# ktiwary2/nerf_pl

Hardware: AMD Instinct MI355X
Metric: rays/sec (64c+128f) Blender-lego 400^2 training step (higher is better)
Workload: dtype f16x3

## Files before the change

__graft_entry__.py:

```python
import os
import subprocess
import sys

REPO = os.path.dirname(os.path.abspath(__file__))


def build() -> None:
    jobs = str(min(16, os.cpu_count() or 1))
    subprocess.run(["make", "-C", REPO, "-j", jobs], check=True)
    r = subprocess.run(["make", "-C", REPO, "-j", jobs, "asan"], check=False)
    if r.returncode != 0:
        print(f"build(): optional `make asan` failed (rc {r.returncode}); "
              "tests/test_abi_asan.py will skip", file=sys.stderr)
    if REPO not in sys.path:
        sys.path.insert(0, REPO)
    import nerf_pl_amd
    from nerf_pl_amd import (_lib, _lib_mesh, _lib_mesh_normals, _lib_optim, _lib_posegrad,
                             _lib_raygrad)
    missing = (_lib.missing_symbols() + _lib_mesh.missing_symbols()
               + _lib_mesh_normals.missing_symbols() + _lib_raygrad.missing_symbols()
               + _lib_posegrad.missing_symbols() + _lib_optim.missing_symbols())
    if missing:
        raise RuntimeError(f"libnerf_pl_amd.so lacks {missing}")


def smoke() -> None:
    if REPO not in sys.path:
        sys.path.insert(0, REPO)
    import torch
    from nerf_pl_amd import Embedding, NeRF, ReplayRNG, render_rays
    from nerf_pl_amd.rays import blender_rays
    from oracle import nerf_oracle as O

    dev = torch.device("cuda", 0)
    n_rays, S, I = 64, 32, 32
    rays = blender_rays(16, 1, near=2.0, far=6.0)[:n_rays].contiguous()
    g = torch.Generator().manual_seed(0)
    draws = [torch.rand(n_rays, S, generator=g), torch.randn(n_rays, S, generator=g),
             torch.rand(n_rays, I, generator=g), torch.rand(n_rays, I, generator=g),
             torch.randn(n_rays, S + I, generator=g)]
    params = [O.make_params(1, sigma_bias=0.5), O.make_params(2, sigma_bias=0.5)]
    ocap, cap = {}, {}
    ref = O.render_rays(params, rays, S, False, 1.0, 1.0, I, 32768, False,
                        rng=O.ReplayRNG(draws), capture=ocap)
# ... 26 lines not shown
```

nerf_pl_amd/csrc/mlp_fwd3.hip:

```cpp
#include "x3.h"

namespace {

using namespace x3;

constexpr int kHeadBytes = NR_H_SIZE * 4;
constexpr int kHeadDma = (kHeadBytes + 1023) / 1024;
constexpr int kHeadLds = kHeadDma * 1024;
#define NR_PE_REGS (NR_F16 || NR_BF1)
constexpr int kPeQ = 12;
constexpr int kPeBytes = NR_PE_REGS ? 0 : kWaves * kPeQ * 64 * 16;
constexpr int kNS = 2;
constexpr int kBlocks = kWaves;
constexpr int kLdsBytes = kRingBytes + kHeadLds + kPeBytes;
static_assert(kLdsBytes <= 160 * 1024, "LDS budget");

constexpr int kL1 = 0, kL2 = 4, kL3 = 20, kL4 = 36, kL5 = 52, kL6 = 72, kL7 = 88, kL8 = 104;
constexpr int kFinal = 120, kDir = 136, kQAll = 145, kQSigma = 120;

struct FwdTab {
    __host__ __device__ static constexpr int64_t off(int q) {
        return (int64_t)kHeadBytes + (int64_t)q * kSlotBytes;
    }
    __host__ __device__ static constexpr int sg(int q) { return q < kDir ? q / 2 : kDir / 2 + (q - kDir); }
    __host__ __device__ static constexpr int first(int G) { return G < kDir / 2 ? 2 * G : kDir + (G - kDir / 2); }
    __host__ __device__ static constexpr int size(int G) { return G < kDir / 2 ? 2 : 1; }
};
static_assert(FwdTab::off(kQAll) == (NR_F16 ? 2388000 : (NR_BF1 ? 1200160 : 3575840)),
              "packed size must match packing.fwd3_offsets()");

template <bool RELU, int NF, int NS>
__device__ __forceinline__ void head_dot(const f32x4 (&acc)[NF][NS], const float* __restrict__ w,
                                         int g, float (&p)[2]) {
    p[0] = p[1] = 0.f;
#pragma unroll
    for (int F = 0; F < NF; ++F) {
        const f32x4 v = *reinterpret_cast<const f32x4*>(w + 16 * F + 4 * g);
#pragma unroll
        for (int S = 0; S < NS; ++S)
#pragma unroll
            for (int r = 0; r < 4; ++r) p[S] = fmaf(RELU ? relu_keep(acc[F][S][r]) : acc[F][S][r], v[r], p[S]);
    }
#pragma unroll
    for (int S = 0; S < NS; ++S) p[S] = sum_over_groups(p[S]);
}

__device__ __forceinline__ void pe_encode(float (&pe)[16], float px, float py, float pz, int g) {
#pragma unroll
    for (int s = 0; s < 2; ++s)
#pragma unroll
        for (int i = 0; i < 4; ++i) {
            const int m = 4 * (4 * s + g) + i;
            const int k = (m * 11) >> 5;
            const int c = m - 3 * k;
            const float v = c == 0 ? px : (c == 1 ? py : pz);
            float sn, cs;
            sincosf(v * __uint_as_float((uint32_t)(127 + k) << 23), &sn, &cs);
            pe[8 * s + i] = sn;
            pe[8 * s + 4 + i] = cs;
        }
    if (g == 3) {
        pe[10] = px; pe[11] = py; pe[14] = pz; pe[15] = 0.f;
    }
}

__device__ __forceinline__ void pe_gather(float (&pe)[16], const float* __restrict__ row, int g) {
#pragma unroll
    for (int s = 0; s < 2; ++s)
#pragma unroll
        for (int i = 0; i < 4; ++i) {
            const int m = min(4 * (4 * s + g) + i, 29);
            const int k = (m * 11) >> 5;
            const int c = m - 3 * k;
            pe[8 * s + i] = row[3 + 6 * k + c];
            pe[8 * s + 4 + i] = row[6 + 6 * k + c];
        }
    if (g == 3) {
        pe[10] = row[0]; pe[11] = row[1]; pe[14] = row[2]; pe[15] = 0.f;
    }
}

__device__ __forceinline__ void dir_encode(float (&d)[8], float dx, float dy, float dz, int g) {
    const float sc = __uint_as_float((uint32_t)(127 + g) << 23);
    sincosf(dx * sc, &d[0], &d[4]);
    sincosf(dy * sc, &d[1], &d[5]);
    sincosf(dz * sc, &d[2], &d[6]);
    d[3] = g == 0 ? dx : (g == 1 ? dy : (g == 2 ? dz : 0.f));
    d[7] = 0.f;
}

__device__ __forceinline__ void dir_gather(float (&d)[8], const float* __restrict__ row, int g) {
#pragma unroll
    for (int c = 0; c < 3; ++c) {
        d[c] = row[3 + 6 * g + c];
        d[4 + c] = row[6 + 6 * g + c];
    }
    d[3] = g < 3 ? row[min(g, 2)] : 0.f;
    d[7] = 0.f;
}

template <int W, bool ROWS>
__device__ __forceinline__ void store_pe4(const float* v, int s, int jh, int S, int g,
                                          float* __restrict__ blk, int lane) {
    const int T = 2 * s + (g >> 1), gp = 2 * (g & 1) + jh;
#if NR_BF1
    store_slot(f32x4{v[0], v[1], v[2], v[3]}, blk, (T * 2 + S) * 64 + 16 * gp + (lane & 15));
#else
    if constexpr (ROWS)
        *reinterpret_cast<f32x4*>(blk + (16 * S + (lane & 15)) * W + 16 * T + 4 * gp) =
            f32x4{v[0], v[1], v[2], v[3]};
    else
// ... 24 lines not shown
template <bool SAVE>
struct DirPeSide {
    static constexpr int before(int T) { return SAVE ? T / 2 : 0; }
    const float (&dpe)[kNS][8];
    float* dst;
    int g, lane;
    template <typename GC>
    __device__ __forceinline__ void operator()(GC, int t) const {
        if constexpr (SAVE) {
            if (t & 1) {
                const int u = t >> 1;
                store_pe4<32, true>(&dpe[u >> 1][4 * (u & 1)], 0, u & 1, u >> 1, g, dst, lane);
            }
        }
    }
};

struct Fwd3Args {
    const char* packed;
    const float* pts; const float* rays; const float* z; const float* x;
    int n, spr, xstride;
    float* out; float* save;
    const int32_t* slist; const int32_t* scount;
};

template <bool RELU, bool STORE, bool MASK, bool SIG, bool ROWS = true>
struct AccU {
    static constexpr bool kStores = STORE;
    static constexpr bool kPaired = STORE && ROWS && kRowPair;
    template <typename P> __device__ __forceinline__ void begin(const P&) {}
    const f32x4 (&X)[16][kNS];
    float* dst;
    uint32_t* msk;
    const float* wsig;
    int lane, g;
    float pend[2] = {0.f, 0.f};
    f32x4 held = {0.f, 0.f, 0.f, 0.f};
    uint32_t w[4] = {0u, 0u, 0u, 0u};
    float sig[2] = {0.f, 0.f};
    f32x2 wsg[2][4];
    __device__ __forceinline__ f32x2 wsig_of(int s, int p) const {
        return *reinterpret_cast<const f32x2*>(wsig + 32 * s + 16 * (p >> 1) + 4 * g + 2 * (p & 1));
    }
    __device__ __forceinline__ void preload() {
        if constexpr (SIG)
#pragma unroll
// ... 45 lines not shown
    const float (&pe)[kNS][N];
    template <typename SC>
    __device__ __forceinline__ void operator()(SC, int sb, int p, float& x0, float& x1) const {
        constexpr int s = SC::value;
        x0 = pe[sb][8 * s + 2 * p];
        x1 = pe[sb][8 * s + 2 * p + 1];
    }
};

template <int S = 0, typename GetU>
__device__ __forceinline__ void drain_all(GetU& u) {
    if constexpr (S < 8) {
#pragma unroll
        for (int sb = 0; sb < kNS; ++sb)
#pragma unroll
            for (int p = 0; p < 4; ++p) {
                float x0, x1;
                u(IC<S>(), sb, p, x0, x1);
            }
        drain_all<S + 1>(u);
    }
}

template <int MODE, bool SIGMA_ONLY, bool SAVE, bool LIST = false>
__global__ void __launch_bounds__(64 * kWaves, 1) mlp_fwd3_kernel(Fwd3Args a) {
    constexpr bool EMB = MODE == FWD_EMB;
    constexpr int QEND = SIGMA_ONLY ? kQSigma : kQAll;
    static_assert(!LIST || (SAVE && MODE == FWD_RAYS), "a listed run saves, on the ray path");
    __shared__ __attribute__((aligned(16))) char smem[kLdsBytes];
    const int lane = threadIdx.x & 63;
    const int wave = __builtin_amdgcn_readfirstlane(threadIdx.x >> 6);
    const int g = lane >> 4;
    const int blk = blockIdx.x * kBlocks + wave;
    const int m = LIST ? __builtin_amdgcn_readfirstlane(*a.scount) : a.n;
    if (LIST && (int)blockIdx.x * kBlocks * 32 >= m) return;
    int smp[2];
    bool valid[2];
#pragma unroll
    for (int S = 0; S < kNS; ++S) {
        const int s_raw = blk * 32 + 16 * S + (lane & 15);
        valid[S] = s_raw < m;
        if constexpr (LIST) smp[S] = a.slist[valid[S] ? s_raw : 0];
        else smp[S] = valid[S] ? s_raw : a.n - 1;
    }
    const char* P = a.packed;

    float pe[kNS][16], dg[kNS][8];
    float in[kNS][7];
#pragma unroll
    for (int S = 0; S < kNS; ++S) {
        const int s = smp[S];
        if constexpr (EMB) {
            pe_gather(pe[S], a.x + (size_t)s * a.xstride, g);
            if constexpr (!SIGMA_ONLY) dir_gather(dg[S], a.x + (size_t)s * a.xstride + NR_XYZ_CH, g);
        } else if constexpr (MODE == FWD_PTS) {
#pragma unroll
            for (int c = 0; c < 3; ++c) in[S][c] = a.pts[(size_t)s * 3 + c];
        } else {
            const float* r = a.rays + (size_t)(s / a.spr) * 8;
#pragma unroll
            for (int c = 0; c < 6; ++c) in[S][c] = r[c];
            in[S][6] = a.z[s];
        }
    }

    float* Hs = reinterpret_cast<float*>(smem + kRingBytes);
    const Dma dma = make_dma(P, FwdTab::off(kQAll), smem, wave, lane);
#pragma unroll
    for (int i = wave; i < kHeadDma; i += kWaves)
        __builtin_amdgcn_raw_ptr_buffer_load_lds(
            dma.rsrc, (__attribute__((address_space(3))) void*)(smem + kRingBytes + i * 1024), 16,
            dma.voff, i * 1024, 0, 0);
    prologue<FwdTab, QEND>(dma);
    const float* H = Hs;
    const int nb = (int)nr_blocks_pad(a.n);
    float* const SV = a.save;

    [[maybe_unused]] f32x4* pe_lds =
        reinterpret_cast<f32x4*>(smem + kRingBytes + kHeadLds) + wave * kPeQ * 64 + lane;
#pragma unroll
    for (int S = 0; S < kNS; ++S) {
        if constexpr (MODE == FWD_PTS) {
            pe_encode(pe[S], in[S][0], in[S][1], in[S][2], g);
        } else if constexpr (MODE == FWD_RAYS) {
            const float zz = in[S][6];
            pe_encode(pe[S], nr_add(in[S][0], nr_mul(in[S][3], zz)),
                      nr_add(in[S][1], nr_mul(in[S][4], zz)), nr_add(in[S][2], nr_mul(in[S][5], zz)), g);
            if constexpr (!SIGMA_ONLY) dir_encode(dg[S], in[S][3], in[S][4], in[S][5], g);
        }
    }
#if !NR_PE_REGS
#pragma unroll
    for (int q = 0; q < 8; ++q)
        pe_lds[q * 64] = f32x4{pe[q >> 2][4 * (q & 3)], pe[q >> 2][4 * (q & 3) + 1],
                               pe[q >> 2][4 * (q & 3) + 2], pe[q >> 2][4 * (q & 3) + 3]};
    if constexpr (!SIGMA_ONLY) {
#pragma unroll
        for (int S = 0; S < 2; ++S) {
            pe_lds[(8 + 2 * S) * 64] = f32x4{dg[S][0], dg[S][1], dg[S][2], dg[S][3]};
            pe_lds[(9 + 2 * S) * 64] = f32x4{dg[S][4], dg[S][5], dg[S][6], dg[S][7]};
        }
    }
#endif

    Ahead f0;
    enter<FwdTab, 0, QEND>(smem, lane, f0);

    ActN<kNS> A, B;
    Pieces b[kNS];
    auto hseg = [&](int l) { return SV + nr_sv_h(l, nb) + (size_t)blk * NR_SEGF(256); };
    NoSide none;
// ... 168 lines not shown
#elif NR_BF1
#define NR_FWD3_BYTES_NAME nr_fwd3_packed_bytes_b1
#else
#define NR_FWD3_BYTES_NAME nr_fwd3_packed_bytes
#endif
NR_API int64_t NR_FWD3_BYTES_NAME(void) { return FwdTab::off(kQAll); }

NR_API int NR_X3_NAME(nr_pack)(const float* flat, const int32_t* map, int64_t n, const int32_t* head_map,
                      void* out, void* stream) {
    NR_REQUIRE(n == (FwdTab::off(kQAll) - kHeadBytes) / 2, "nr_pack_x3: map has %lld entries, "
               "expected %lld", (long long)n, (long long)((FwdTab::off(kQAll) - kHeadBytes) / 2));
    NR_REQUIRE(flat && map && head_map && out, "nr_pack_x3: null pointer");
    pack3_kernel<<<(unsigned)((n + 255) / 256), 256, 0, (hipStream_t)stream>>>(
        flat, map, n, head_map, reinterpret_cast<char*>(out));
    NR_LAUNCH_CHECK("nr_pack_x3");
    return 0;
}

NR_API int NR_X3_NAME(nr_mlp_fwd)(const void* packed, const float* rays, const float* z, int64_t n,
                         int samples_per_ray, const float* x, int xstride, int sigma_only,
                         float* out, float* save, void* stream) {
    NR_REQUIRE(n >= 0 && n < (int64_t)1 << 31, "nr_mlp_fwd_x3: n=%lld out of range", (long long)n);
    if (n == 0) return 0;
    NR_REQUIRE(packed && out, "nr_mlp_fwd_x3: null packed/out");
    NR_REQUIRE(((uintptr_t)packed & 15) == 0 && ((uintptr_t)out & 15) == 0 &&
                   ((uintptr_t)save & 15) == 0,
               "nr_mlp_fwd_x3: packed/out/save must be 16-byte aligned");
    const bool emb = x != nullptr;
    if (emb) {
        NR_REQUIRE(xstride >= (sigma_only ? NR_XYZ_CH : NR_XYZ_CH + NR_DIR_CH),
                   "nr_mlp_fwd_x3: xstride %d too small", xstride);
    } else {
        NR_REQUIRE(rays && z && samples_per_ray > 0, "nr_mlp_fwd_x3: rays/z/samples_per_ray");
    }
    NR_REQUIRE(!(sigma_only && save && emb),
               "nr_mlp_fwd_x3: a sigma_only run keeps activations only on the ray path");
    Fwd3Args a{reinterpret_cast<const char*>(packed), nullptr, rays, z, x, (int)n,
               samples_per_ray, xstride, out, save};
    const int blocks = (int)((n + 32 * kBlocks - 1) / (32 * kBlocks));
    hipStream_t st = (hipStream_t)stream;
    const bool sv = save != nullptr;
    if (emb) {
        if (sigma_only) mlp_fwd3_kernel<FWD_EMB, true, false><<<blocks, 64 * kWaves, 0, st>>>(a);
        else if (sv) mlp_fwd3_kernel<FWD_EMB, false, true><<<blocks, 64 * kWaves, 0, st>>>(a);
        else mlp_fwd3_kernel<FWD_EMB, false, false><<<blocks, 64 * kWaves, 0, st>>>(a);
    } else {
        if (sigma_only && sv) mlp_fwd3_kernel<FWD_RAYS, true, true><<<blocks, 64 * kWaves, 0, st>>>(a);
        else if (sigma_only) mlp_fwd3_kernel<FWD_RAYS, true, false><<<blocks, 64 * kWaves, 0, st>>>(a);
        else if (sv) mlp_fwd3_kernel<FWD_RAYS, false, true><<<blocks, 64 * kWaves, 0, st>>>(a);
        else mlp_fwd3_kernel<FWD_RAYS, false, false><<<blocks, 64 * kWaves, 0, st>>>(a);
    }
    NR_LAUNCH_CHECK("nr_mlp_fwd_x3");
    return 0;
}

#if !NR_BF1
NR_API int NR_X3_NAME(nr_mlp_fwd_listed)(const void* packed, const float* rays, const float* z,
                                         int64_t n, int samples_per_ray, int sigma_only,
                                         float* save, const int32_t* samples,
                                         const int32_t* count, void* stream) {
    NR_REQUIRE(n >= 0 && n < (int64_t)1 << 31, "nr_mlp_fwd_listed: n=%lld out of range", (long long)n);
    if (n == 0) return 0;
    NR_REQUIRE(packed && rays && z && save && samples && count && samples_per_ray > 0,
               "nr_mlp_fwd_listed: null pointer or samples_per_ray");
    NR_REQUIRE(((uintptr_t)packed & 15) == 0 && ((uintptr_t)save & 15) == 0,
               "nr_mlp_fwd_listed: packed/save must be 16-byte aligned");
    Fwd3Args a{reinterpret_cast<const char*>(packed), nullptr, rays, z, nullptr, (int)n,
               samples_per_ray, 0, nullptr, save, samples, count};
    const int blocks = (int)((n + 32 * kBlocks - 1) / (32 * kBlocks));
    hipStream_t st = (hipStream_t)stream;
    if (sigma_only) mlp_fwd3_kernel<FWD_RAYS, true, true, true><<<blocks, 64 * kWaves, 0, st>>>(a);
    else mlp_fwd3_kernel<FWD_RAYS, false, true, true><<<blocks, 64 * kWaves, 0, st>>>(a);
    NR_LAUNCH_CHECK("nr_mlp_fwd_listed");
    return 0;
}
#endif

NR_API int NR_X3_NAME(nr_mlp_sigma_points)(const void* packed, const float* pts, int64_t n,
                                  float* sigma_out, void* stream) {
// ... 12 lines not shown
```

nerf_pl_amd/csrc/probe.hip:

```cpp
#include "layout.h"

NR_API int64_t nr_layout_query(int what) {
    switch (what) {
        case 0: return NR_F_TOTAL;
        case 1: return NR_F_HEAD;
        case 2: return NR_B_TOTAL;
        case 3: return NR_SAVE_PER_BLOCK;
        case 4: return NR_GRAD_PER_BLOCK;
        case 5: return NR_H_SIZE;
        case 6: return NR_F_L5;
        case 7: return NR_F_DIR;
        case 8: return NR_B_L5T;
        case 9: return 2;
        default: return -1;
    }
}

namespace {
__global__ void probe_mfma_kernel(const float* a_in, const float* b_in, float* d_out) {
    const int l = threadIdx.x;
    const float a = a_in[(l & 31) * 2 + (l >> 5)];
    const float b = b_in[(l >> 5) * 32 + (l & 31)];
    f32x16 c = {};
    c = nr_mfma32(a, b, c);
    for (int r = 0; r < 16; ++r) d_out[nr_acc_row(r, l >> 5) * 32 + (l & 31)] = c[r];
}

__global__ void probe_rand_kernel(uint64_t seed, uint32_t stream, uint64_t idx0, int64_t n,
                                  float* __restrict__ uniform_out,
                                  float* __restrict__ normal_out) {
    const int64_t i = (int64_t)blockIdx.x * blockDim.x + threadIdx.x;
    if (i >= n) return;
    if (uniform_out) uniform_out[i] = nr_rand_uniform(seed, stream, idx0 + (uint64_t)i);
    if (normal_out) normal_out[i] = nr_rand_normal(seed, stream, idx0 + (uint64_t)i);
}
}
// ... 17 lines not shown
```

nerf_pl_amd/functions.py:

```python
from __future__ import annotations

import collections
import functools
import os
import threading
import weakref

import torch

from . import ops, packing
from ._lib import call, stream_of


@functools.lru_cache(maxsize=4)
def _wgrad_workspace(device_index: int, stream: int = 0) -> torch.Tensor:
    from ._lib import lib
    nbytes = int(lib().nr_wgrad_workspace_bytes(0))
    return torch.empty(nbytes // 4, dtype=torch.float32, device=torch.device("cuda", device_index))


SIGMA_TRAIN_KERNELS = os.environ.get("NERF_PL_AMD_SIGMA_TRAIN", "1") != "0"

ACTIVE_SAMPLES = os.environ.get("NERF_PL_AMD_ACTIVE_SAMPLES", "1") != "0"
ACTIVE_ARITHS = ("f16x3", "bf16x6", "fp32")
# ... 32 lines not shown
    host = torch.empty(1, dtype=torch.int32, pin_memory=True)
    host.copy_(count_dev, non_blocking=True)
    ev = torch.cuda.Event()
    ev.record()
    with _LISTED_LOCK:
        per_model = _LISTED.get(model)
        if per_model is None:
            per_model = _LISTED[model] = {}
        per_model.setdefault(sigma_only, _ListedStats()).pending.append((host, ev, n))


ACTIVE_LOG = None

_DEBUG = {} if os.environ.get("NERF_PL_AMD_DEBUG") == "1" else None

_SHAPES = list(packing.param_shapes().items())
_SIGMA_ONLY_UNUSED = {"xyz_encoding_final.weight", "xyz_encoding_final.bias",
                      "dir_encoding.0.weight", "dir_encoding.0.bias",
                      "rgb.0.weight", "rgb.0.bias"}


class _FusedMLP(torch.autograd.Function):
    @staticmethod
    def forward(ctx, model, rays, z, spr, x, sigma_only, *params):
        train = any(ctx.needs_input_grad[6:])
        ray_grad = x is None and (ctx.needs_input_grad[1] or ctx.needs_input_grad[2])
        bwd = train or ray_grad
        if train and sigma_only and x is not None:
            raise NotImplementedError("nerf_pl_amd: training NeRF.forward(x, sigma_only=True) on "
                                      "pre-embedded input is not supported; use render_rays")
        packed_f, packed_b = model.packed(backward=bwd)
        so_train = bwd and sigma_only and SIGMA_TRAIN_KERNELS and x is None
        kern_sigma_only = sigma_only and (not bwd or so_train)
        defer = False
        if bwd and x is None and ACTIVE_SAMPLES and ops.arith_of(packed_b) in ACTIVE_ARITHS:
            if DEFER_SAVE == "all" or (DEFER_SAVE in ("sigma", "auto") and so_train):
                defer = True
            elif DEFER_SAVE == "auto":
                frac = _listed_fraction(model, sigma_only)
                defer = frac is not None and frac < DEFER_AUTO
        model.__dict__["_nr_defer_last"] = defer
        if x is None:
            rays = ops._dev(rays, "rays", 8)
            z = ops._dev(z, "z")
        out, save = ops.mlp_forward(packed_f, rays=rays, z=z, samples_per_ray=spr, x=x,
                                    sigma_only=kern_sigma_only, save=bwd and not defer)
        if _DEBUG is not None and save is not None:
            _DEBUG.setdefault("fwd_saves", []).append((save, out.shape[0], ops.MATH))
        if bwd:
            flat = model.flat_params()
            if defer:
                ctx.save_for_backward(out, rays, z, packed_f, packed_b, flat, *params)
            else:
                ctx.save_for_backward(out, save, packed_f, packed_b, flat, *params,
                                      *((rays, z) if ray_grad else ()))
            ctx.spr = spr
            ctx.train, ctx.ray_grad = train, ray_grad
            ctx.defer = defer
            ctx.sigma_only = sigma_only
            ctx.model = model if DEFER_SAVE == "auto" else None
            ctx.so_kernels = so_train
        if sigma_only and bwd and out.shape[1] == 4:
            out = out[:, 3:4].contiguous()
        return out

    @staticmethod
    def backward(ctx, g_out):
        if ctx.defer:
            out, rays, z, packed_f, packed_b, flat = ctx.saved_tensors[:6]
            n, mode = z.numel(), "_listed"
        else:
            out, save, packed_f, packed_b, flat = ctx.saved_tensors[:5]
            n = out.shape[0]
            mode = "_active" if ACTIVE_SAMPLES and ops.arith_of(packed_b) in ACTIVE_ARITHS else ""
        dev = out.device
        if ctx.sigma_only:
            g4 = torch.zeros(n, 4, device=dev)
            g4[:, 3:4] = g_out
            g_out = g4
        g_out = g_out.contiguous()
        if out.shape[1] != 4:
            out = g_out
        so = ctx.so_kernels
        sfx = ("_sigma" if so else "") + mode
        st = stream_of(dev)
        lst = ()
        if mode:
            sl = _sample_list(ctx, g_out, n, st)
            lst = (sl.data_ptr(), sl.data_ptr() + 4 * n)
        if ctx.defer:
            save = torch.empty(ops.save_floats(n), device=dev)
            call(ops.entry("nr_mlp_fwd_listed", packed_f), packed_f.data_ptr(), rays.data_ptr(),
                 z.data_ptr(), n, int(ctx.spr), int(so), save.data_ptr(), *lst, st)
        grad_ws = torch.empty(ops.n_blocks(n) * ops.GRAD_PER_BLOCK, device=dev)
        call(ops.entry("nr_mlp_bwd" + sfx, packed_b), packed_b.data_ptr(), ops.head_ptr(packed_f),
             out.data_ptr(), g_out.data_ptr(), save.data_ptr(), n, grad_ws.data_ptr(), *lst, st)
        gflat = None
        if ctx.train:
            gflat = torch.empty(packing.N_PARAMS, device=dev)
            ws = _wgrad_workspace(dev.index, int(st))
            call(ops.entry("nr_wgrad" + sfx, packed_b), save.data_ptr(), grad_ws.data_ptr(), n,
                 ws.data_ptr(), gflat.data_ptr(), *lst, st)
            if not so:
                _dir_feat(flat, gflat, st)
        g_rays = g_z = None
        if ctx.ray_grad:
            if not ctx.defer:
                rays, z = ctx.saved_tensors[-2:]
            g_rays, g_smp = ops.mlp_ray_gradient(flat, grad_ws, rays, z, int(ctx.spr),
                                                 ops.arith_of(packed_b), so, lst)
            g_rays = g_rays if ctx.needs_input_grad[1] else None
            g_z = g_smp[:, 3] if ctx.needs_input_grad[2] else None
        if _DEBUG is not None:
            _DEBUG.update(save=save, grad_ws=grad_ws, g_out=g_out, gflat=gflat, n=n)
            _DEBUG.setdefault("g_outs", []).append(g_out)
        pgrads = _param_grads(gflat, ctx.sigma_only) if ctx.train else (None,) * len(_SHAPES)
        return (None, g_rays, g_z, None, None, None) + pgrads


def _sample_list(ctx, g_out, n, st):
    sl = torch.empty(n + 1 + 2 * ((n + 31) // 32), dtype=torch.int32, device=g_out.device)
    call("nr_active_samples", g_out.data_ptr(), n, sl.data_ptr(), sl.data_ptr() + 4 * n,
         sl.data_ptr() + 4 * (n + 1), st)
    if ACTIVE_LOG is not None:
        ACTIVE_LOG.append((sl, n))
    if ctx.model is not None:
        _note_listed(ctx.model, ctx.sigma_only, sl[n:n + 1], n)
    return sl


def _dir_feat(flat, gflat, st):
    call("nr_wgrad_dir_feat", flat.data_ptr(), gflat.data_ptr(), st)


def _param_grads(gflat, sigma_only):
    grads, off = [], 0
    for name, shp in _SHAPES:
        k = 1
        for d in shp:
            k *= d
        g = gflat[off:off + k].view(shp)
        off += k
        grads.append(None if (sigma_only and name in _SIGMA_ONLY_UNUSED) else g)
    return tuple(grads)


def mlp_apply(model, *, rays=None, z=None, spr=0, x=None, sigma_only=False):
    if x is not None and x.requires_grad:
        raise NotImplementedError("nerf_pl_amd: gradients w.r.t. the embedded input are not "
                                  "produced (the reference never needs them)")
    params = model.ordered_params()
    if z is not None:
        z = z.reshape(-1)
    ray_grad = x is None and any(t is not None and t.requires_grad for t in (rays, z))
    if not (any(p.requires_grad for p in params) or ray_grad) or not torch.is_grad_enabled():
        packed_f, _ = model.packed()
        out, _ = ops.mlp_forward(packed_f, rays=rays, z=z, samples_per_ray=spr, x=x,
                                 sigma_only=sigma_only)
        return out
    return _FusedMLP.apply(model, rays, z, spr, x, sigma_only, *params)


class _Composite(torch.autograd.Function):

    @staticmethod
    def forward(ctx, raw, z, rays, noise, noise_std, seed, stream, white_back, disp):
        outs = ops.composite_forward(raw, z, rays, noise, noise_std, seed, stream, white_back,
                                     disp=disp)
        ctx.save_for_backward(raw, z, rays, noise if noise is not None else torch.empty(0),
                              *(outs[1:3] if disp else ()))
        ctx.cfg = (noise is not None, noise_std, seed, stream, white_back, disp)
        ctx.mark_non_differentiable(outs[-1])
        ctx.set_materialize_grads(False)
        return outs

    @staticmethod
    def backward(ctx, *g):
        raw, z, rays, noise = ctx.saved_tensors[:4]
        has_noise, noise_std, seed, stream, white_back, disp = ctx.cfg
        noise = noise if has_noise else None
        g_raw = g_z = g_rays = None
        if ctx.needs_input_grad[0]:
            g_raw = ops.composite_backward(raw, z, rays, noise, noise_std, seed, stream,
# ... 66 lines not shown
```

nerf_pl_amd/ops.py:

```python
from __future__ import annotations

import functools
import os

import numpy as np
import torch

from . import packing
from ._lib import call, lib, ptr, stream_of

BLK = 32
MATHS = ("f16x3", "bf16x6", "fp32", "bf16")
MATH = os.environ.get("NERF_PL_AMD_MATH", "f16x3")
if MATH not in MATHS:
    raise ValueError(f"NERF_PL_AMD_MATH must be one of {MATHS}, got {MATH!r}")
SAVE_PER_BLOCK = BLK * (64 + 8 * 256 + 128 + 32) + 9 * 256
SAVE_STATS, STAT_SEGS = 16, 11


_LAYOUT_OK = False
ABI_REVISION = 2


def _check_layout():
    global _LAYOUT_OK
    if not _LAYOUT_OK:
        q = lib().nr_layout_query
        got = (int(q(3)), int(q(4)), int(q(9)))
        want = (SAVE_PER_BLOCK, GRAD_PER_BLOCK, ABI_REVISION)
        if got != want:
            raise RuntimeError(f"nerf_pl_amd: libnerf_pl_amd.so has (save block, grad block, ABI "
                               f"revision) {got}, the package {want}: rebuild the library (make)")
        _LAYOUT_OK = True


def save_floats(n: int) -> int:
    _check_layout()
    nb = n_blocks(n)
    return nb * SAVE_PER_BLOCK + SAVE_STATS + STAT_SEGS * nb
GRAD_PER_BLOCK = BLK * (8 * 256 + 128 + 4)


def n_blocks(n: int) -> int:
    return (n + 4 * BLK - 1) // (4 * BLK) * 4
FWD_PACKED = packing.layer_offsets(packing.FWD_LAYERS)[1] + packing.HEAD_SIZE
BWD_PACKED = packing.layer_offsets(packing.BWD_LAYERS)[1]


def _dev(t: torch.Tensor, name: str, shape_last=None):
# ... 100 lines not shown
    return torch.from_numpy(packing.build_bwd3_map(np_)).to(torch.device("cuda", device_index))


def pack_bwd(flat: torch.Tensor, out: torch.Tensor | None = None, math: str | None = None):
    math = math or MATH
    if math in _SUFFIX:
        np_ = packing.NPIECES[math]
        m = _map_bwd3(flat.device.index, np_)
        out = torch.empty(packing.bwd3_bytes(np_), dtype=torch.uint8, device=flat.device) \
            if out is None else out
        call("nr_pack_bwd" + _SUFFIX[math], ptr(flat), ptr(m), m.numel(), ptr(out),
             stream_of(flat.device))
        return out
    return pack_bwd_fp32(flat, out)


def pack_bwd_fp32(flat: torch.Tensor, out: torch.Tensor | None = None) -> torch.Tensor:
    _, m = _maps(flat.device.index)
    out = torch.empty(BWD_PACKED, device=flat.device) if out is None else out
    call("nr_pack", ptr(flat), ptr(m), m.numel(), ptr(out), stream_of(flat.device))
    return out


def mlp_forward(packed: torch.Tensor, *, rays=None, z=None, samples_per_ray=0, x=None,
                sigma_only=False, save=False):
    if x is not None:
        x = _dev(x, "x")
        n, xstride = x.shape[0], x.shape[1]
    else:
        rays = _dev(rays, "rays", 8)
        z = _dev(z, "z")
        n, xstride = z.numel(), 0
    dev = packed.device
    out = torch.empty(n, 1 if sigma_only and not save else 4, device=dev)
    sv = torch.empty(save_floats(n), device=dev) if save else None
    call(entry("nr_mlp_fwd", packed), ptr(packed), ptr(rays), ptr(z), n, int(samples_per_ray),
         ptr(x), xstride, int(sigma_only), ptr(out), ptr(sv), stream_of(dev))
    return out, sv


def sigma_points(packed, pts):
    pts = _dev(pts, "pts", 3)
    out = torch.empty(pts.shape[0], device=pts.device)
    call(entry("nr_mlp_sigma_points", packed), ptr(packed), ptr(pts), pts.shape[0], ptr(out),
         stream_of(pts.device))
    return out


def coarse_z(rays, n_samples, use_disp, perturb, u=None, seed=0):
    rays = _dev(rays, "rays", 8)
    n_rays = rays.shape[0]
    z = torch.empty(n_rays, n_samples, device=rays.device)
    tl = linspace_table(n_samples, rays.device.index)
    call("nr_coarse_z", ptr(rays), ptr(tl), n_rays, n_samples, int(use_disp), float(perturb),
         ptr(u), seed, ptr(z), stream_of(rays.device))
    return z


def composite_forward(raw, z, rays, noise, noise_std, seed, rng_stream, white_back,
                      weights_only=False, disp=False):
    if disp and weights_only:
# ... 162 lines not shown
```

nerf_pl_amd/rendering.py:

```python
from __future__ import annotations

import functools
import os

import torch

from . import ops
from .functions import coarse_z_apply, composite_apply, merged_z_apply, mlp_apply
from .rng import (STREAM_JITTER, STREAM_NOISE_COARSE, STREAM_NOISE_FINE, STREAM_PERTURB,
                  STREAM_U, PhiloxRNG, TorchRNG)

__all__ = ["render_rays", "sample_pdf"]

FINE_STREAM = os.environ.get("NERF_PL_AMD_FINE_STREAM", "1") != "0"
FINE_STREAM_PRIORITY = int(os.environ.get("NERF_PL_AMD_FINE_STREAM_PRIORITY", "0"))


BEFORE_FINE = []


@functools.lru_cache(maxsize=None)
def _side_stream(device_index: int):
    return torch.cuda.Stream(device=torch.device("cuda", device_index),
                             priority=FINE_STREAM_PRIORITY)
# ... 49 lines not shown
    return _render_rays(models, embeddings, rays, N_samples, use_disp, perturb, noise_std,
                        N_importance, chunk, white_back, test_time, rng, _capture)


def _render_rays(models, embeddings, rays, N_samples, use_disp, perturb, noise_std, N_importance,
                 chunk, white_back, test_time, rng, _capture, disp=False, depth_only=False,
                 pipelined=True, empty_ok=False):
    if isinstance(rays, torch.Tensor) and rays.device.type == "cpu":
        if depth_only:
            raise NotImplementedError("nerf_pl_amd.render_rays: depth_only needs a HIP-device batch")
        if rays.dtype != torch.float32:
            raise TypeError(f"rays: expected float32, got {rays.dtype}")
        if rays.dim() != 2 or rays.shape[-1] != 8:
            raise ValueError(f"rays: expected (N, 8), got {tuple(rays.shape)}")
        from .host import render_rays_host
        return render_rays_host(models, embeddings, rays, N_samples, use_disp, perturb, noise_std,
                                N_importance, chunk, white_back, test_time,
                                TorchRNG() if rng is None else rng, _capture, disp=disp)
    del chunk
    fused = _fused_ok(models, embeddings)

    def mlp(model, z, spr, sigma_only=False):
        if fused:
            return mlp_apply(model, rays=rays, z=z, spr=spr, sigma_only=sigma_only)
        return _composable_mlp(model, embeddings, rays, z, spr, sigma_only)

    rays = ops._dev(rays, "rays", 8)
    if not fused and rays.requires_grad and torch.is_grad_enabled():
        raise NotImplementedError(
            "nerf_pl_amd.render_rays: the composable path (a non-default NeRF or Embedding) does "
            "not produce the gradient with respect to the rays; detach them, or use the default "
            "NeRF() with [Embedding(3, 10), Embedding(3, 4)]")
    dev = rays.device
    n_rays = rays.shape[0]
    if n_rays == 0 and not empty_ok:
        raise ValueError("nerf_pl_amd.render_rays: empty ray batch (the reference's "
                         "inference() concatenates an empty chunk list, rendering.py:161)")
    rng = PhiloxRNG() if rng is None else rng
    seed = rng.seed

    def composite(result, level, raw, z, noise, stream):
        rgb, depth, opac, *dmap, w = composite_apply(raw, z, rays, noise, noise_std, seed, stream,
                                                     white_back, disp)
        if rgb is not None:
            result["rgb_" + level] = rgb
        result["depth_" + level] = depth
        result["opacity_" + level] = opac
        if disp:
            result["disp_map_" + level] = dmap[0]
        return w
# ... 22 lines not shown
        jit = rng.rand((n_rays, N_importance), dev)
        z_f = merged_z_apply(z_c, w_c.detach(), rays, N_importance, u, jit, seed)
        cap["z_fine"] = z_f
        s_f = N_samples + N_importance

        fine = {}

        def fine_pass():
            noise_f = rng.randn((n_rays, s_f), dev)
            raw_f = mlp(models[1], z_f, s_f, sigma_only=depth_only)
            w = composite(fine, "fine", raw_f, z_f, noise_f, STREAM_NOISE_FINE)
            return tuple(fine.values()) + (w,)

        while pipelined and BEFORE_FINE:
            BEFORE_FINE.pop(0)()
        if pipelined and FINE_STREAM and torch.is_grad_enabled() and any(
                p.requires_grad for p in models[1].parameters()):
            main = torch.cuda.current_stream(dev)
            side = _side_stream(dev.index)
            side.wait_stream(main)
            with torch.cuda.stream(side):
                outs = fine_pass()
            main.wait_stream(side)
            for t in (rays, z_f):
                t.record_stream(side)
            for t in outs:
                t.record_stream(main)
        else:
            outs = fine_pass()
        cap["weights_fine"] = outs[-1]
        result.update(fine)
    return result


_STREAMS = (STREAM_PERTURB, STREAM_NOISE_COARSE, STREAM_U, STREAM_JITTER, STREAM_NOISE_FINE)
```

Baseline: 531,200.

## Precompute per-ray direction encoding table and use a bounded-argument sincos fast path

Adds a small kernel that encodes each ray's view direction (sin/cos at four frequencies) once per ray into a table. The ray-path MLP forward kernels, including the deferred listed recompute in backward, read this table instead of evaluating sincos for every sample. Separately, the positional encoding checks per wave whether all sample coordinates are small and, if so, calls sincos with an assumed bounded argument so the compiler can drop the large-argument reduction path. The cost is an extra launch, a per-ray table held in memory and saved for backward, and a wave-wide ballot branch, plus a probe kernel that checks the fast sincos is bit-identical.

```diff
diff --git a/__graft_entry__.py b/__graft_entry__.py
--- a/__graft_entry__.py
+++ b/__graft_entry__.py
@@ -15,11 +15,12 @@
     if REPO not in sys.path:
         sys.path.insert(0, REPO)
     import nerf_pl_amd
-    from nerf_pl_amd import (_lib, _lib_mesh, _lib_mesh_normals, _lib_optim, _lib_posegrad,
-                             _lib_raygrad)
+    from nerf_pl_amd import (_lib, _lib_dirtab, _lib_mesh, _lib_mesh_normals, _lib_optim,
+                             _lib_posegrad, _lib_raygrad)
     missing = (_lib.missing_symbols() + _lib_mesh.missing_symbols()
                + _lib_mesh_normals.missing_symbols() + _lib_raygrad.missing_symbols()
-               + _lib_posegrad.missing_symbols() + _lib_optim.missing_symbols())
+               + _lib_posegrad.missing_symbols() + _lib_optim.missing_symbols()
+               + _lib_dirtab.missing_symbols())
     if missing:
         raise RuntimeError(f"libnerf_pl_amd.so lacks {missing}")
 
diff --git a/include/nerf_pl_amd_dirtab.h b/include/nerf_pl_amd_dirtab.h
--- /dev/null
+++ b/include/nerf_pl_amd_dirtab.h
@@ -0,0 +1,39 @@
+#ifndef NERF_PL_AMD_DIRTAB_H
+#define NERF_PL_AMD_DIRTAB_H
+
+#include <stdint.h>
+
+#ifdef __cplusplus
+extern "C" {
+#endif
+
+#define NR_XSTRIDE_DIR_TABLE (-32)
+
+int nr_dir_encode(const float* rays, int64_t n_rays, float* table, void* stream);
+
+int nr_mlp_fwd_dirtab_x3(const void* packed, const float* rays, const float* z, int64_t n,
+                         int samples_per_ray, int sigma_only, float* out, float* save,
+                         const float* dir_table, void* stream);
+int nr_mlp_fwd_dirtab_h3(const void* packed, const float* rays, const float* z, int64_t n,
+                         int samples_per_ray, int sigma_only, float* out, float* save,
+                         const float* dir_table, void* stream);
+int nr_mlp_fwd_dirtab_b1(const void* packed, const float* rays, const float* z, int64_t n,
+                         int samples_per_ray, int sigma_only, float* out, float* save,
+                         const float* dir_table, void* stream);
+
+int nr_mlp_fwd_listed_dirtab_x3(const void* packed, const float* rays, const float* z, int64_t n,
+                                int samples_per_ray, int sigma_only, float* save,
+                                const int32_t* samples, const int32_t* count,
+                                const float* dir_table, void* stream);
+int nr_mlp_fwd_listed_dirtab_h3(const void* packed, const float* rays, const float* z, int64_t n,
+                                int samples_per_ray, int sigma_only, float* save,
+                                const int32_t* samples, const int32_t* count,
+                                const float* dir_table, void* stream);
+
+int nr_probe_sincos_small(int64_t first_bits, int64_t count, uint64_t* result, void* stream);
+
+#ifdef __cplusplus
+}
+#endif
+
+#endif
diff --git a/nerf_pl_amd/_lib_dirtab.py b/nerf_pl_amd/_lib_dirtab.py
--- /dev/null
+++ b/nerf_pl_amd/_lib_dirtab.py
@@ -0,0 +1,48 @@
+from __future__ import annotations
+
+import ctypes
+
+from . import _lib
+
+_p = ctypes.c_void_p
+_i = ctypes.c_int
+_i64 = ctypes.c_int64
+
+_FWD = [_p, _p, _p, _i64, _i, _i, _p, _p, _p, _p]
+_FWD_LISTED = [_p, _p, _p, _i64, _i, _i, _p, _p, _p, _p, _p]
+XSTRIDE_DIR_TABLE = -32
+
+SIGNATURES = {
+    "nr_dir_encode": [_p, _i64, _p, _p],
+    **{"nr_mlp_fwd_dirtab" + s: _FWD for s in ("_x3", "_h3", "_b1")},
+    **{"nr_mlp_fwd_listed_dirtab" + s: _FWD_LISTED for s in ("_x3", "_h3")},
+    "nr_probe_sincos_small": [_i64, _i64, _p, _p],
+}
+RESTYPES = {}
+
+_bound = None
+
+
+def lib():
+    global _bound
+    if _bound is None:
+        L = _lib.lib()
+        for name, args in SIGNATURES.items():
+            fn = getattr(L, name, None)
+            if fn is None:
+                continue
+            fn.argtypes = args
+            fn.restype = RESTYPES.get(name, _i)
+        _bound = L
+    return _bound
+
+
+def missing_symbols() -> list:
+    L = lib()
+    return [n for n in SIGNATURES if getattr(L, n, None) is None]
+
+
+def call(name: str, *args) -> None:
+    rc = getattr(lib(), name)(*args)
+    if rc != 0:
+        raise RuntimeError(f"{name} failed (code {rc}): {_lib.last_error()}")
diff --git a/nerf_pl_amd/csrc/dirtab.hip b/nerf_pl_amd/csrc/dirtab.hip
--- /dev/null
+++ b/nerf_pl_amd/csrc/dirtab.hip
@@ -0,0 +1,71 @@
+#include "pe.h"
+
+namespace {
+
+__global__ void __launch_bounds__(256) dir_table_kernel(const float* __restrict__ rays,
+                                                        int64_t n_rays, float* __restrict__ table) {
+    const int64_t t = (int64_t)blockIdx.x * blockDim.x + threadIdx.x;
+    if (t >= n_rays * 4) return;
+    const float* r = rays + (t >> 2) * 8;
+    float d[8];
+    dir_encode(d, r[3], r[4], r[5], (int)(t & 3));
+    f32x4* o = reinterpret_cast<f32x4*>(table + t * 8);
+    o[0] = f32x4{d[0], d[1], d[2], d[3]};
+    o[1] = f32x4{d[4], d[5], d[6], d[7]};
+}
+
+__device__ __attribute__((noinline)) void sincos_library(float x, float* sn, float* cs) {
+    sincosf(x, sn, cs);
+}
+
+__global__ void __launch_bounds__(256) probe_sincos_kernel(uint32_t first, int64_t count,
+                                                           unsigned long long* __restrict__ result) {
+    const int64_t stride = (int64_t)gridDim.x * blockDim.x;
+    unsigned long long bad = 0, where = ~0ull;
+    for (int64_t i = (int64_t)blockIdx.x * blockDim.x + threadIdx.x; i < count; i += stride) {
+        const uint32_t bits = first + (uint32_t)i;
+#pragma unroll
+        for (int sign = 0; sign < 2; ++sign) {
+            const float x = __uint_as_float(bits | ((uint32_t)sign << 31));
+            float s0, c0, s1, c1;
+            sincos_library(x, &s0, &c0);
+            sincos_arg<true>(x, &s1, &c1);
+            if (__float_as_uint(s0) != __float_as_uint(s1) || __float_as_uint(c0) != __float_as_uint(c1)) {
+                ++bad;
+                where = where < bits ? where : bits;
+            }
+        }
+    }
+    if (bad) {
+        atomicAdd(result, bad);
+        atomicMin(result + 1, where);
+    }
+}
+
+}
+
+NR_API int nr_dir_encode(const float* rays, int64_t n_rays, float* table, void* stream) {
+    NR_REQUIRE(n_rays >= 0 && n_rays < (int64_t)1 << 29, "nr_dir_encode: n_rays=%lld out of range",
+               (long long)n_rays);
+    if (n_rays == 0) return 0;
+    NR_REQUIRE(rays && table, "nr_dir_encode: null pointer");
+    NR_REQUIRE(((uintptr_t)table & 15) == 0, "nr_dir_encode: table must be 16-byte aligned");
+    dir_table_kernel<<<(unsigned)((n_rays * 4 + 255) / 256), 256, 0, (hipStream_t)stream>>>(
+        rays, n_rays, table);
+    NR_LAUNCH_CHECK("nr_dir_encode");
+    return 0;
+}
+
+NR_API int nr_probe_sincos_small(int64_t first_bits, int64_t count, uint64_t* result, void* stream) {
+    NR_REQUIRE(first_bits >= 0 && count >= 0 &&
+                   first_bits + count <= (int64_t)__builtin_bit_cast(uint32_t, kSinCosSmall),
+               "nr_probe_sincos_small: patterns [%lld, +%lld) reach the bound 2^17",
+               (long long)first_bits, (long long)count);
+    NR_REQUIRE(result, "nr_probe_sincos_small: null result");
+    if (count == 0) return 0;
+    const int64_t blocks = (count + 256 * 1024 - 1) / (256 * 1024);
+    probe_sincos_kernel<<<(unsigned)blocks, 256, 0, (hipStream_t)stream>>>(
+        (uint32_t)first_bits, count, reinterpret_cast<unsigned long long*>(result));
+    NR_LAUNCH_CHECK("nr_probe_sincos_small");
+    return 0;
+}
diff --git a/nerf_pl_amd/csrc/mlp_fwd3.hip b/nerf_pl_amd/csrc/mlp_fwd3.hip
--- a/nerf_pl_amd/csrc/mlp_fwd3.hip
+++ b/nerf_pl_amd/csrc/mlp_fwd3.hip
@@ -1,4 +1,5 @@
 #include "x3.h"
+#include "pe.h"
 
 namespace {
 
@@ -45,6 +46,7 @@
     for (int S = 0; S < NS; ++S) p[S] = sum_over_groups(p[S]);
 }
 
+template <bool SMALL = false>
 __device__ __forceinline__ void pe_encode(float (&pe)[16], float px, float py, float pz, int g) {
 #pragma unroll
     for (int s = 0; s < 2; ++s)
@@ -55,7 +57,7 @@
             const int c = m - 3 * k;
             const float v = c == 0 ? px : (c == 1 ? py : pz);
             float sn, cs;
-            sincosf(v * __uint_as_float((uint32_t)(127 + k) << 23), &sn, &cs);
+            sincos_arg<SMALL>(v * __uint_as_float((uint32_t)(127 + k) << 23), &sn, &cs);
             pe[8 * s + i] = sn;
             pe[8 * s + 4 + i] = cs;
         }
@@ -78,15 +80,6 @@
     if (g == 3) {
         pe[10] = row[0]; pe[11] = row[1]; pe[14] = row[2]; pe[15] = 0.f;
     }
-}
-
-__device__ __forceinline__ void dir_encode(float (&d)[8], float dx, float dy, float dz, int g) {
-    const float sc = __uint_as_float((uint32_t)(127 + g) << 23);
-    sincosf(dx * sc, &d[0], &d[4]);
-    sincosf(dy * sc, &d[1], &d[5]);
-    sincosf(dz * sc, &d[2], &d[6]);
-    d[3] = g == 0 ? dx : (g == 1 ? dy : (g == 2 ? dz : 0.f));
-    d[7] = 0.f;
 }
 
 __device__ __forceinline__ void dir_gather(float (&d)[8], const float* __restrict__ row, int g) {
@@ -157,6 +150,7 @@
     int n, spr, xstride;
     float* out; float* save;
     const int32_t* slist; const int32_t* scount;
+    const float* dirtab;
 };
 
 template <bool RELU, bool STORE, bool MASK, bool SIG, bool ROWS = true>
@@ -248,9 +242,10 @@
     }
 }
 
-template <int MODE, bool SIGMA_ONLY, bool SAVE, bool LIST = false>
+template <int MODE, bool SIGMA_ONLY, bool SAVE, bool LIST = false, bool TAB = false>
 __global__ void __launch_bounds__(64 * kWaves, 1) mlp_fwd3_kernel(Fwd3Args a) {
     constexpr bool EMB = MODE == FWD_EMB;
+    static_assert(!TAB || (MODE == FWD_RAYS && !SIGMA_ONLY), "the table feeds the dir layer of the ray path");
     constexpr int QEND = SIGMA_ONLY ? kQSigma : kQAll;
     static_assert(!LIST || (SAVE && MODE == FWD_RAYS), "a listed run saves, on the ray path");
     __shared__ __attribute__((aligned(16))) char smem[kLdsBytes];
@@ -283,10 +278,17 @@
 #pragma unroll
             for (int c = 0; c < 3; ++c) in[S][c] = a.pts[(size_t)s * 3 + c];
         } else {
-            const float* r = a.rays + (size_t)(s / a.spr) * 8;
+            const int ray = s / a.spr;
+            const float* r = a.rays + (size_t)ray * 8;
 #pragma unroll
             for (int c = 0; c < 6; ++c) in[S][c] = r[c];
             in[S][6] = a.z[s];
+            if constexpr (TAB) {
+                const f32x4* t = reinterpret_cast<const f32x4*>(a.dirtab + (size_t)ray * 32 + 8 * g);
+                const f32x4 lo = t[0], hi = t[1];
+#pragma unroll
+                for (int e = 0; e < 4; ++e) { dg[S][e] = lo[e]; dg[S][4 + e] = hi[e]; }
+            }
         }
     }
 
@@ -304,15 +306,26 @@
 
     [[maybe_unused]] f32x4* pe_lds =
         reinterpret_cast<f32x4*>(smem + kRingBytes + kHeadLds) + wave * kPeQ * 64 + lane;
-#pragma unroll
-    for (int S = 0; S < kNS; ++S) {
-        if constexpr (MODE == FWD_PTS) {
-            pe_encode(pe[S], in[S][0], in[S][1], in[S][2], g);
-        } else if constexpr (MODE == FWD_RAYS) {
-            const float zz = in[S][6];
-            pe_encode(pe[S], nr_add(in[S][0], nr_mul(in[S][3], zz)),
-                      nr_add(in[S][1], nr_mul(in[S][4], zz)), nr_add(in[S][2], nr_mul(in[S][5], zz)), g);
-            if constexpr (!SIGMA_ONLY) dir_encode(dg[S], in[S][3], in[S][4], in[S][5], g);
+    if constexpr (!EMB) {
+        float pt[kNS][3];
+        bool small = true;
+#pragma unroll
+        for (int S = 0; S < kNS; ++S) {
+#pragma unroll
+            for (int c = 0; c < 3; ++c) {
+                if constexpr (MODE == FWD_PTS) pt[S][c] = in[S][c];
+                else pt[S][c] = nr_add(in[S][c], nr_mul(in[S][3 + c], in[S][6]));
+                small = small && __builtin_fabsf(pt[S][c]) * 512.f < kSinCosSmall;
+            }
+            if constexpr (MODE == FWD_RAYS && !SIGMA_ONLY && !TAB)
+                dir_encode(dg[S], in[S][3], in[S][4], in[S][5], g);
+        }
+        if (__builtin_amdgcn_ballot_w64(!small) == 0) {
+#pragma unroll
+            for (int S = 0; S < kNS; ++S) pe_encode<true>(pe[S], pt[S][0], pt[S][1], pt[S][2], g);
+        } else {
+#pragma unroll
+            for (int S = 0; S < kNS; ++S) pe_encode<false>(pe[S], pt[S][0], pt[S][1], pt[S][2], g);
         }
     }
 #if !NR_PE_REGS
@@ -527,6 +540,14 @@
                          float* out, float* save, void* stream) {
     NR_REQUIRE(n >= 0 && n < (int64_t)1 << 31, "nr_mlp_fwd_x3: n=%lld out of range", (long long)n);
     if (n == 0) return 0;
+    const float* dir_table = nullptr;
+    if (xstride == NR_XSTRIDE_DIR_TABLE) {
+        NR_REQUIRE(((uintptr_t)x & 15) == 0, "nr_mlp_fwd_x3: dir_table must be 16-byte aligned");
+        NR_REQUIRE(x || sigma_only, "nr_mlp_fwd_x3: null dir_table");
+        dir_table = sigma_only ? nullptr : x;
+        x = nullptr;
+        xstride = 0;
+    }
     NR_REQUIRE(packed && out, "nr_mlp_fwd_x3: null packed/out");
     NR_REQUIRE(((uintptr_t)packed & 15) == 0 && ((uintptr_t)out & 15) == 0 &&
                    ((uintptr_t)save & 15) == 0,
@@ -541,11 +562,14 @@
     NR_REQUIRE(!(sigma_only && save && emb),
                "nr_mlp_fwd_x3: a sigma_only run keeps activations only on the ray path");
     Fwd3Args a{reinterpret_cast<const char*>(packed), nullptr, rays, z, x, (int)n,
-               samples_per_ray, xstride, out, save};
+               samples_per_ray, xstride, out, save, nullptr, nullptr, dir_table};
     const int blocks = (int)((n + 32 * kBlocks - 1) / (32 * kBlocks));
     hipStream_t st = (hipStream_t)stream;
     const bool sv = save != nullptr;
-    if (emb) {
+    if (dir_table) {
+        if (sv) mlp_fwd3_kernel<FWD_RAYS, false, true, false, true><<<blocks, 64 * kWaves, 0, st>>>(a);
+        else mlp_fwd3_kernel<FWD_RAYS, false, false, false, true><<<blocks, 64 * kWaves, 0, st>>>(a);
+    } else if (emb) {
         if (sigma_only) mlp_fwd3_kernel<FWD_EMB, true, false><<<blocks, 64 * kWaves, 0, st>>>(a);
         else if (sv) mlp_fwd3_kernel<FWD_EMB, false, true><<<blocks, 64 * kWaves, 0, st>>>(a);
         else mlp_fwd3_kernel<FWD_EMB, false, false><<<blocks, 64 * kWaves, 0, st>>>(a);
@@ -559,7 +583,39 @@
     return 0;
 }
 
+NR_API int NR_X3_NAME(nr_mlp_fwd_dirtab)(const void* packed, const float* rays, const float* z,
+                                         int64_t n, int samples_per_ray, int sigma_only,
+                                         float* out, float* save, const float* dir_table,
+                                         void* stream) {
+    return NR_X3_NAME(nr_mlp_fwd)(packed, rays, z, n, samples_per_ray, dir_table,
+                                  NR_XSTRIDE_DIR_TABLE, sigma_only, out, save, stream);
+}
+
 #if !NR_BF1
+NR_API int NR_X3_NAME(nr_mlp_fwd_listed_dirtab)(const void* packed, const float* rays,
+                                                const float* z, int64_t n, int samples_per_ray,
+                                                int sigma_only, float* save, const int32_t* samples,
+                                                const int32_t* count, const float* dir_table,
+                                                void* stream) {
+    NR_REQUIRE(n >= 0 && n < (int64_t)1 << 31, "nr_mlp_fwd_listed_dirtab: n=%lld out of range",
+               (long long)n);
+    if (n == 0) return 0;
+    NR_REQUIRE(packed && rays && z && save && samples && count && samples_per_ray > 0,
+               "nr_mlp_fwd_listed_dirtab: null pointer or samples_per_ray");
+    NR_REQUIRE(sigma_only || dir_table, "nr_mlp_fwd_listed_dirtab: null dir_table");
+    NR_REQUIRE(((uintptr_t)packed & 15) == 0 && ((uintptr_t)save & 15) == 0 &&
+                   ((uintptr_t)dir_table & 15) == 0,
+               "nr_mlp_fwd_listed_dirtab: packed/save/dir_table must be 16-byte aligned");
+    Fwd3Args a{reinterpret_cast<const char*>(packed), nullptr, rays, z, nullptr, (int)n,
+               samples_per_ray, 0, nullptr, save, samples, count, dir_table};
+    const int blocks = (int)((n + 32 * kBlocks - 1) / (32 * kBlocks));
+    hipStream_t st = (hipStream_t)stream;
+    if (sigma_only) mlp_fwd3_kernel<FWD_RAYS, true, true, true><<<blocks, 64 * kWaves, 0, st>>>(a);
+    else mlp_fwd3_kernel<FWD_RAYS, false, true, true, true><<<blocks, 64 * kWaves, 0, st>>>(a);
+    NR_LAUNCH_CHECK("nr_mlp_fwd_listed_dirtab");
+    return 0;
+}
+
 NR_API int NR_X3_NAME(nr_mlp_fwd_listed)(const void* packed, const float* rays, const float* z,
                                          int64_t n, int samples_per_ray, int sigma_only,
                                          float* save, const int32_t* samples,
diff --git a/nerf_pl_amd/csrc/pe.h b/nerf_pl_amd/csrc/pe.h
--- /dev/null
+++ b/nerf_pl_amd/csrc/pe.h
@@ -0,0 +1,21 @@
+#pragma once
+#include "common.h"
+
+#define NR_XSTRIDE_DIR_TABLE (-32)
+
+constexpr float kSinCosSmall = 131072.f;
+
+template <bool SMALL>
+__device__ __forceinline__ void sincos_arg(float x, float* sn, float* cs) {
+    if constexpr (SMALL) __builtin_assume(__builtin_fabsf(x) < kSinCosSmall);
+    sincosf(x, sn, cs);
+}
+
+__device__ __forceinline__ void dir_encode(float (&d)[8], float dx, float dy, float dz, int g) {
+    const float sc = __uint_as_float((uint32_t)(127 + g) << 23);
+    sincosf(dx * sc, &d[0], &d[4]);
+    sincosf(dy * sc, &d[1], &d[5]);
+    sincosf(dz * sc, &d[2], &d[6]);
+    d[3] = g == 0 ? dx : (g == 1 ? dy : (g == 2 ? dz : 0.f));
+    d[7] = 0.f;
+}
diff --git a/nerf_pl_amd/csrc/probe.hip b/nerf_pl_amd/csrc/probe.hip
--- a/nerf_pl_amd/csrc/probe.hip
+++ b/nerf_pl_amd/csrc/probe.hip
@@ -11,7 +11,7 @@
         case 6: return NR_F_L5;
         case 7: return NR_F_DIR;
         case 8: return NR_B_L5T;
-        case 9: return 2;
+        case 9: return 3;
         default: return -1;
     }
 }
diff --git a/nerf_pl_amd/functions.py b/nerf_pl_amd/functions.py
--- a/nerf_pl_amd/functions.py
+++ b/nerf_pl_amd/functions.py
@@ -78,8 +78,8 @@
 
 class _FusedMLP(torch.autograd.Function):
     @staticmethod
-    def forward(ctx, model, rays, z, spr, x, sigma_only, *params):
-        train = any(ctx.needs_input_grad[6:])
+    def forward(ctx, model, rays, z, spr, x, sigma_only, dir_table, *params):
+        train = any(ctx.needs_input_grad[7:])
         ray_grad = x is None and (ctx.needs_input_grad[1] or ctx.needs_input_grad[2])
         bwd = train or ray_grad
         if train and sigma_only and x is not None:
@@ -100,19 +100,22 @@
             rays = ops._dev(rays, "rays", 8)
             z = ops._dev(z, "z")
         out, save = ops.mlp_forward(packed_f, rays=rays, z=z, samples_per_ray=spr, x=x,
-                                    sigma_only=kern_sigma_only, save=bwd and not defer)
+                                    sigma_only=kern_sigma_only, save=bwd and not defer,
+                                    dir_table=dir_table)
         if _DEBUG is not None and save is not None:
             _DEBUG.setdefault("fwd_saves", []).append((save, out.shape[0], ops.MATH))
         if bwd:
             flat = model.flat_params()
             if defer:
-                ctx.save_for_backward(out, rays, z, packed_f, packed_b, flat, *params)
+                ctx.save_for_backward(out, rays, z, packed_f, packed_b, flat, *params,
+                                      *(() if dir_table is None else (dir_table,)))
             else:
                 ctx.save_for_backward(out, save, packed_f, packed_b, flat, *params,
                                       *((rays, z) if ray_grad else ()))
             ctx.spr = spr
             ctx.train, ctx.ray_grad = train, ray_grad
             ctx.defer = defer
+            ctx.has_table = dir_table is not None
             ctx.sigma_only = sigma_only
             ctx.model = model if DEFER_SAVE == "auto" else None
             ctx.so_kernels = so_train
@@ -145,9 +148,8 @@
             sl = _sample_list(ctx, g_out, n, st)
             lst = (sl.data_ptr(), sl.data_ptr() + 4 * n)
         if ctx.defer:
-            save = torch.empty(ops.save_floats(n), device=dev)
-            call(ops.entry("nr_mlp_fwd_listed", packed_f), packed_f.data_ptr(), rays.data_ptr(),
-                 z.data_ptr(), n, int(ctx.spr), int(so), save.data_ptr(), *lst, st)
+            table = ctx.saved_tensors[-1] if ctx.has_table else None
+            save = ops.mlp_forward_listed(packed_f, rays, z, ctx.spr, so, *lst, dir_table=table)
         grad_ws = torch.empty(ops.n_blocks(n) * ops.GRAD_PER_BLOCK, device=dev)
         call(ops.entry("nr_mlp_bwd" + sfx, packed_b), packed_b.data_ptr(), ops.head_ptr(packed_f),
              out.data_ptr(), g_out.data_ptr(), save.data_ptr(), n, grad_ws.data_ptr(), *lst, st)
@@ -171,7 +173,7 @@
             _DEBUG.update(save=save, grad_ws=grad_ws, g_out=g_out, gflat=gflat, n=n)
             _DEBUG.setdefault("g_outs", []).append(g_out)
         pgrads = _param_grads(gflat, ctx.sigma_only) if ctx.train else (None,) * len(_SHAPES)
-        return (None, g_rays, g_z, None, None, None) + pgrads
+        return (None, g_rays, g_z, None, None, None, None) + pgrads
 
 
 def _sample_list(ctx, g_out, n, st):
@@ -201,7 +203,7 @@
     return tuple(grads)
 
 
-def mlp_apply(model, *, rays=None, z=None, spr=0, x=None, sigma_only=False):
+def mlp_apply(model, *, rays=None, z=None, spr=0, x=None, sigma_only=False, dir_table=None):
     if x is not None and x.requires_grad:
         raise NotImplementedError("nerf_pl_amd: gradients w.r.t. the embedded input are not "
                                   "produced (the reference never needs them)")
@@ -212,9 +214,9 @@
     if not (any(p.requires_grad for p in params) or ray_grad) or not torch.is_grad_enabled():
         packed_f, _ = model.packed()
         out, _ = ops.mlp_forward(packed_f, rays=rays, z=z, samples_per_ray=spr, x=x,
-                                 sigma_only=sigma_only)
+                                 sigma_only=sigma_only, dir_table=dir_table)
         return out
-    return _FusedMLP.apply(model, rays, z, spr, x, sigma_only, *params)
+    return _FusedMLP.apply(model, rays, z, spr, x, sigma_only, dir_table, *params)
 
 
 class _Composite(torch.autograd.Function):
diff --git a/nerf_pl_amd/ops.py b/nerf_pl_amd/ops.py
--- a/nerf_pl_amd/ops.py
+++ b/nerf_pl_amd/ops.py
@@ -19,12 +19,14 @@
 
 
 _LAYOUT_OK = False
-ABI_REVISION = 2
+ABI_REVISION = 3
 
 
 def _check_layout():
     global _LAYOUT_OK
     if not _LAYOUT_OK:
+        from . import _lib_dirtab
+        _lib_dirtab.lib()
         q = lib().nr_layout_query
         got = (int(q(3)), int(q(4)), int(q(9)))
         want = (SAVE_PER_BLOCK, GRAD_PER_BLOCK, ABI_REVISION)
@@ -171,8 +173,21 @@
     return out
 
 
+def dir_encode(rays: torch.Tensor) -> torch.Tensor:
+    _check_layout()
+    rays = _dev(rays, "rays", 8)
+    table = torch.empty(rays.shape[0], 32, device=rays.device)
+    call("nr_dir_encode", ptr(rays), rays.shape[0], ptr(table), stream_of(rays.device))
+    return table
+
+
+def has_dir_table(packed_or_math) -> bool:
+    a = packed_or_math if isinstance(packed_or_math, str) else arith_of(packed_or_math)
+    return a in _SUFFIX
+
+
 def mlp_forward(packed: torch.Tensor, *, rays=None, z=None, samples_per_ray=0, x=None,
-                sigma_only=False, save=False):
+                sigma_only=False, save=False, dir_table=None):
     if x is not None:
         x = _dev(x, "x")
         n, xstride = x.shape[0], x.shape[1]
@@ -183,9 +198,32 @@
     dev = packed.device
     out = torch.empty(n, 1 if sigma_only and not save else 4, device=dev)
     sv = torch.empty(save_floats(n), device=dev) if save else None
+    if dir_table is not None:
+        from ._lib_dirtab import XSTRIDE_DIR_TABLE
+        if x is not None or not has_dir_table(packed):
+            raise ValueError("nerf_pl_amd: dir_table goes with the ray path of a split-operand "
+                             f"arithmetic (got {'x' if x is not None else arith_of(packed)})")
+        dir_table = _dev(dir_table, "dir_table", 32)
+        if dir_table.shape[0] != rays.shape[0]:
+            raise ValueError(f"dir_table: {dir_table.shape[0]} rows for {rays.shape[0]} rays")
+        x, xstride = dir_table, XSTRIDE_DIR_TABLE
     call(entry("nr_mlp_fwd", packed), ptr(packed), ptr(rays), ptr(z), n, int(samples_per_ray),
          ptr(x), xstride, int(sigma_only), ptr(out), ptr(sv), stream_of(dev))
     return out, sv
+
+
+def mlp_forward_listed(packed, rays, z, samples_per_ray, sigma_only, samples, count,
+                       dir_table=None):
+    n, dev = z.numel(), packed.device
+    save = torch.empty(save_floats(n), device=dev)
+    if dir_table is not None:
+        call(entry("nr_mlp_fwd_listed_dirtab", packed), ptr(packed), ptr(rays), ptr(z), n,
+             int(samples_per_ray), int(sigma_only), ptr(save), samples, count, ptr(dir_table),
+             stream_of(dev))
+    else:
+        call(entry("nr_mlp_fwd_listed", packed), ptr(packed), ptr(rays), ptr(z), n,
+             int(samples_per_ray), int(sigma_only), ptr(save), samples, count, stream_of(dev))
+    return save
 
 
 def sigma_points(packed, pts):
diff --git a/nerf_pl_amd/rendering.py b/nerf_pl_amd/rendering.py
--- a/nerf_pl_amd/rendering.py
+++ b/nerf_pl_amd/rendering.py
@@ -95,10 +95,14 @@
 
     def mlp(model, z, spr, sigma_only=False):
         if fused:
-            return mlp_apply(model, rays=rays, z=z, spr=spr, sigma_only=sigma_only)
+            return mlp_apply(model, rays=rays, z=z, spr=spr, sigma_only=sigma_only,
+                             dir_table=dir_table)
         return _composable_mlp(model, embeddings, rays, z, spr, sigma_only)
 
     rays = ops._dev(rays, "rays", 8)
+    dir_table = None
+    if fused and not depth_only and rays.shape[0] and ops.has_dir_table(ops.MATH):
+        dir_table = ops.dir_encode(rays.detach())
     if not fused and rays.requires_grad and torch.is_grad_enabled():
         raise NotImplementedError(
             "nerf_pl_amd.render_rays: the composable path (a non-default NeRF or Embedding) does "
@@ -167,7 +171,7 @@
             with torch.cuda.stream(side):
                 outs = fine_pass()
             main.wait_stream(side)
-            for t in (rays, z_f):
+            for t in (rays, z_f) + (() if dir_table is None else (dir_table,)):
                 t.record_stream(side)
             for t in outs:
                 t.record_stream(main)
```

Result: no change. 531,000 (-0.0%).
